# AVianEco/Softspoken

Measured on AMD Instinct MI355X. Metric: audio-seconds processed/sec (whole node), 16 kHz mono, higher is better.
Workload: dtype f16x2

## Files before the change

### softspoken_amd/csrc/conv4.hip

```cpp
#include "conv4_forms.h"
#include <cstdio>
#include <cstdlib>
#include <type_traits>
#include <utility>

namespace ss {

static constexpr int kMfmaPrio = 2;
__device__ __forceinline__ uint32_t relu_pk(uint32_t v) {
    return __builtin_bit_cast(uint32_t, __builtin_elementwise_max(__builtin_bit_cast(s16x2, v), s16x2{0, 0}));
}
__device__ __forceinline__ uint32_t max_pk(uint32_t a, uint32_t b) {
    return __builtin_bit_cast(uint32_t, __builtin_elementwise_max(__builtin_bit_cast(s16x2, a), __builtin_bit_cast(s16x2, b)));
}

template <int NT, int NW, bool BRES, bool RES, bool RADD, bool POOL, int RP, bool FIRST, bool FLAT, bool PF2, bool SPLIT = false, bool RANK1 = false,
          int NH = 1, bool GRES = false>
__global__ __launch_bounds__(64 * NW * NH) __attribute__((amdgpu_waves_per_eu((NT <= 2 && !(SPLIT && RES && !BRES && NW == 4 && NH == 1)) ? 4 : 2)))
void conv3x3_v4_kernel(ConvArgs a, int total_tiles, int lds_b_bytes) {
    constexpr int KC = 32;
    constexpr bool DUO = NH > 1;
    static_assert(!DUO || (NT == 1 && NW * NH == 16 && (RP == 0 || (GRES && RP == 1 && POOL)) && !FIRST && !FLAT && !PF2),
                  "DUO: the plain A / B launches; GRES also conv2_1.B's projection in B");
    static_assert(!GRES || (DUO && BRES && SPLIT && !RES), "GRES: f16x2 B launches with resident banks");
// ... 26 lines not shown
    const int hh = lane >> 5, m = lane & 31;
    const int py = (m >> 1) & 1, px = (m & 1) | ((m >> 2) << 1);
    char* sA = smem + half * kA;
    const int sb_bytes = RING ? 2 * lds_b_bytes : lds_b_bytes;
    char* sB = smem + NH * kA;
    const int proj_steps = RP ? (a.C0x + a.C1x) / 16 : 0;
    constexpr bool proj_lds = RP > 0 && (BRES || NT == 3 || SPLIT);
    const char* sProj = smem + NH * kA + sb_bytes;
    const int proj_tiles = SPLIT ? a.Cout / 32 : NT;
    const int proj_bank = proj_steps * proj_tiles * 1024;
    const float* sBias = (const float*)(sProj + (proj_lds ? (SPLIT ? 2 : 1) * proj_bank : 0));
    constexpr int FW = 20, FROWS = PR + 3;
    float* sFb = (float*)sBias + 32;
    float* sF = sFb + 32;
    float* sFlat = (float*)sBias + 32;

    const int H = a.H, W = a.W, Cout = a.Cout;
    const int ngroups = Cout / (32 * NT);
    const int nch_r = (a.C0 + a.C1) / KC;
    const int nch = SPLIT ? 2 * nch_r : nch_r;
    const int all_taps = nch_r * TAPS;

    const int xcd = blockIdx.x & 7, local = (int)(blockIdx.x >> 3) * NH + half, gper = (int)(gridDim.x >> 3) * NH;
    const int per = (total_tiles + 7) >> 3;
#ifdef SS_DEVBUILD
    const bool order_seq = !(a.dbg & 512);
#else
    constexpr bool order_seq = !kOrderSideBySide;
#endif
    auto tile_of = [&](int loc, int it) -> int {
        if constexpr (GRES) {
            const RingItem r = gres_item(xcd, loc / NH, (int)(gridDim.x >> 3), it, loc % NH, total_tiles / ngroups, ngroups, NH);
            return r.pos >= 0 ? r.pos * ngroups + r.g : -1;
        }
        if constexpr (RING) {
            const RingItem r = ring_item(xcd, loc / NH, (int)(gridDim.x >> 3), it, loc % NH, total_tiles / ngroups, ngroups, order_seq);
            return r.pos >= 0 ? r.pos * ngroups + r.g : -1;
        }
        const int idx = loc + it * gper;
        const int t = xcd * per + idx;
        return (idx < per && t < total_tiles) ? t : -1;
    };
    auto tile_at = [&](int it) -> int { return tile_of(local, it); };
    struct Tile { int n, y0, x0, g; };
    auto decode = [&](int t) -> Tile {
        Tile d;
        d.g = t % ngroups; t /= ngroups;
        d.x0 = (t % a.tiles_x) * 16; t /= a.tiles_x;
        d.y0 = (t % a.tiles_y) * TH;
        d.n = t / a.tiles_y;
        return d;
    };

    uint32_t pix_full[AIT], pix_half[AIT], lds_off[AIT], flags = 0;
    const uint32_t part16 = (tid & 3) * 16;
    {
        const int Wh = W >> 1;
#pragma unroll
        for (int it = 0; it < AIT; ++it) {
            const int p = tid + NTHR * it;
            const int pix = p >> 2;
            const int pyy = pix / kPatch, pxx = pix - pyy * kPatch;
            lds_off[it] = pyy * kRowPitch + pxx * kPixPitch + part16;
            pix_full[it] = pyy * W + pxx;
            pix_half[it] = ((pyy + 1) >> 1) * Wh + ((pxx + 1) >> 1);
            const uint32_t f = (pyy == 0 ? 1u : 0u) | (pyy == PR - 1 ? 2u : 0u) | (pxx == 0 ? 4u : 0u) | (pxx == kPatch - 1 ? 8u : 0u) |
                               (p >= NPA ? 16u : 0u);
            flags |= f << (8 * it);
        }
    }
    u32x4 ra0[AIT], ra1[AIT];
    u32x4 rb[BIT];
    float rf = 0.f;
    static_assert(!FIRST || (PR + 2) * FW <= NTHR, "one feature value per thread");

    auto issue_patch = [&](const Tile& d, int ci, u32x4 (&ra)[AIT]) {
        if constexpr (FIRST) {
            if constexpr (SPLIT) { if (ci & 1) return; }
            const int fy = tid / FW, fx = tid - fy * FW;
            const int Y = d.y0 - 2 + fy, X = d.x0 - 2 + fx;
            rf = (tid < (PR + 2) * FW && (unsigned)Y < (unsigned)H && (unsigned)X < (unsigned)W)
                     ? a.rank1_src[((size_t)d.n * H + Y) * W + X] : 0.f;
            return;
        }
        const int ch = (SPLIT ? ci >> 1 : ci) * KC;
        const int64_t plane = (SPLIT && !(ci & 1)) ? a.lo_delta : 0;
        const char* base; uint32_t cs2, toff; bool up;
        if (ch < a.C0) {
            base = (const char*)a.src0 - kHdr + plane; cs2 = 2u * a.C0; up = false;
            toff = kHdr + ((((uint32_t)d.n * H + d.y0 - 1) * W + d.x0 - 1) * a.C0 + ch) * 2u;
        } else {
            base = (const char*)a.src1 - kHdr + plane; cs2 = 2u * a.C1; up = true;
            toff = kHdr + ((((uint32_t)d.n * (H >> 1) + (d.y0 >> 1) - 1) * (W >> 1) + (d.x0 >> 1) - 1) * a.C1 + (ch - a.C0)) * 2u;
        }
        uint32_t tm = (d.y0 == 0 ? 1u : 0u) | (d.y0 + TH == H ? 2u : 0u) | (d.x0 == 0 ? 4u : 0u) | (d.x0 + 16 == W ? 8u : 0u) | 16u;
        const uint32_t tp = toff + part16;
#pragma unroll
        for (int it = 0; it < AIT; ++it) {
            const uint32_t pix = up ? pix_half[it] : pix_full[it];
            uint32_t off = __umul24(pix, cs2) + tp;
            if (flags & (tm << (8 * it))) off = 0;
            ra[it] = *(const u32x4*)(base + off);
        }
    };
    auto issue_weights = [&](const Tile& d, int ci) {
        if constexpr (!BRES && !RING) {
            if constexpr (SPLIT) { if (ci & 1) return; }
            const char* wsrc = SPLIT ? (const char*)a.wpk + ((size_t)d.g * nch_r + (ci >> 1)) * 2 * (TAPS * kTapBytes)
                                     : (const char*)a.wpk + ((size_t)d.g * all_taps + ci * TAPS) * kTapBytes;
#pragma unroll
            for (int it = 0; it < BIT; ++it) {
                const int p = tid + NTHR * it;
                u32x4 v = {0u, 0u, 0u, 0u};
                if (p < NPB) v = *(const u32x4*)(wsrc + p * 16);
                rb[it] = v;
            }
        }
    };
    auto commit = [&](u32x4 (&ra)[AIT], bool patch, bool bank) {
        if constexpr (FIRST) return;
        if (patch) {
#pragma unroll
            for (int it = 0; it < AIT; ++it) {
                if ((it + 1) * NTHR <= NPA || !(flags & (16u << (8 * it)))) *(u32x4*)(sA + lds_off[it]) = ra[it];
            }
        }
        if constexpr (!BRES && !RING) {
            if (bank) {
#pragma unroll
                for (int it = 0; it < BIT; ++it) {
                    const int p = tid + NTHR * it;
                    if (p < NPB) *(u32x4*)(sB + p * 16) = rb[it];
                }
            }
        }
    };
    constexpr int NPH = NPB / 2;
    const int ring_g0 = RING ? ring_group0((int)(blockIdx.x >> 3), ngroups, order_seq) : 0;
    const int ring_gstep = RING ? ring_group_step((int)(gridDim.x >> 3), ngroups, order_seq) : 0;
    int ring_g = ring_g0, ring_c = 0;
    auto ring_duty = [&](int s, int n_chunks) {
        if constexpr (RING) {
            if (half > 1) return;
            const int k = (s >> 1) + 1;
            if (k >= n_chunks) return;
            if (!(s & 1)) {
                if (++ring_c == nch_r) { ring_c = 0; ring_g += ring_gstep; if (ring_g >= ngroups) ring_g -= ngroups; }
                const char* wsrc = (const char*)a.wpk + ((size_t)(ring_g * nch_r + ring_c) * 2 + half) * (TAPS * kTapBytes);
#pragma unroll
                for (int it = 0; it < BIT; ++it) {
                    const int p = tid + NTHR * it;
                    u32x4 v = {0u, 0u, 0u, 0u};
// ... 267 lines not shown
                for (int nt = 0; nt < NT; ++nt) { rlo[nt] = *(const u32x4*)(rp + nt * 64); rhi[nt] = *(const u32x4*)(rp + nt * 64 + 32); }
            }
        }
        u32x4 fw[FLAT ? 2 : 1];
        u32x4 fw2[(FLAT && SPLIT) ? 2 : 1];
        auto load_flat_w = [&]() {
#pragma unroll
            for (int sx = 0; sx < 2; ++sx) {
                fw[sx] = *(const u32x4*)((const char*)a.flat_w4 + (((cur.y0 >> 1) + wave) * 2 + sx) * 1024 + lane * 16);
                if constexpr (SPLIT) fw2[sx] = *(const u32x4*)((const char*)a.flat_w4 + 64 * 2 * 1024 + (((cur.y0 >> 1) + wave) * 2 + sx) * 1024 + lane * 16);
            }
        };
        if constexpr (FLAT && !(SPLIT && RP > 0)) load_flat_w();
        u32x4 xf[RP ? RP : 1];
        if constexpr (RP > 0 && !SPLIT) {
            const uint32_t t_full = kHdr + ((((uint32_t)cur.n * H + cur.y0 + 2 * wave) * W + cur.x0) * a.C0x) * 2u;
            const uint32_t t_half = kHdr + ((((uint32_t)cur.n * (H >> 1) + (cur.y0 >> 1) + wave) * (W >> 1) + (cur.x0 >> 1)) * a.C1x) * 2u;
#pragma unroll
            for (int k = 0; k < RP; ++k) {
                const int sidx = ci * RP + k, ch = sidx * 16;
                const char* base; uint32_t off;
                if (sidx >= proj_steps) { base = (const char*)a.xp0 - kHdr; off = 0; }
                else if (ch < a.C0x) { base = (const char*)a.xp0 - kHdr; off = t_full + xf_off + ch * 2u; }
                else { base = (const char*)a.xp1 - kHdr; off = t_half + xh_off + (ch - a.C0x) * 2u; }
                xf[k] = *(const u32x4*)(base + off);
            }
        }
        u32x4 wpg[(RP && !proj_lds) ? RP : 1][NT];
        if constexpr (RP > 0 && !proj_lds && !SPLIT) {
            {
                const int tiles = Cout / 32;
#pragma unroll
                for (int k = 0; k < RP; ++k) {
                    const int sidx = ci * RP + k < proj_steps ? ci * RP + k : 0;
#pragma unroll
                    for (int nt = 0; nt < NT; ++nt)
                        wpg[k][nt] = *(const u32x4*)((const char*)a.proj_w + ((size_t)(sidx * tiles + cur.g * NT + nt) * 64 + lane) * 16);
                }
            }
        }
        if (ci == 0) {
#pragma unroll
            for (int nt = 0; nt < NT; ++nt)
#pragma unroll
                for (int g = 0; g < 4; ++g) {
                    const f32x4 b4 = *(const f32x4*)(sBias + co0 + nt * 32 + 8 * g + 4 * hh);
                    acc[nt][4 * g] = b4[0]; acc[nt][4 * g + 1] = b4[1]; acc[nt][4 * g + 2] = b4[2]; acc[nt][4 * g + 3] = b4[3];
                    if constexpr (RES) {
                        const f32x4 r4 = *(const f32x4*)(sBias + Cout + co0 + nt * 32 + 8 * g + 4 * hh);
                        racc[nt][4 * g] = r4[0]; racc[nt][4 * g + 1] = r4[1]; racc[nt][4 * g + 2] = r4[2]; racc[nt][4 * g + 3] = r4[3];
                    }
                }
        }
        auto proj_products = [&](auto k0c, auto k1c) {
            constexpr int K0 = decltype(k0c)::value, K1 = decltype(k1c)::value;
#pragma unroll
            for (int k = K0; k < K1; ++k) {
                const int sidx = (ci >> 1) * RP + k < proj_steps ? (ci >> 1) * RP + k : 0;
#pragma unroll
                for (int nt = 0; nt < NT; ++nt) {
                    const int wt = (sidx * proj_tiles + (int)(co0 >> 5) + nt) * 1024 + lane * 16;
                    const u32x4 wh = *(const u32x4*)(sProj + wt), wl = *(const u32x4*)(sProj + proj_bank + wt);
                    acc[nt] = mfma16<true>(wh, pxl[k - K0], acc[nt]);
                    acc[nt] = mfma16<true>(wl, pxh[k - K0], acc[nt]);
                    acc[nt] = mfma16<true>(wh, pxh[k - K0], acc[nt]);
                }
            }
        };
        using KZ_ = std::integral_constant<int, 0>; using KH_ = std::integral_constant<int, RPH>; using KR_ = std::integral_constant<int, RP>;
        if constexpr (SPLIT && RP > 0 && PART == 1) {
            proj_products(KZ_{}, KH_{});
            __builtin_amdgcn_sched_barrier(0);
            if constexpr (RP > RPH) issue_proj(cur, ci >> 1, KH_{}, KR_{});
        }
        if constexpr (FLAT && SPLIT && RP > 0) load_flat_w();
        {
            const char* bbase = sB + boff0 + (BRES ? ((DUO && !GRES ? cur.g * nch : 0) + (SPLIT ? (ci >> 1) * 2 : ci)) * TAPS * kTapBytes
                                                   : RING ? ((stage_no >> 1) & 1) * lds_b_bytes : 0);
            constexpr int PD = (NT == 1) ? 4 : 2;
            u32x4 af[PD], bfr[PD][NT];
            u32x4 rfr[RES ? 2 : 1][RES ? NT : 1];
            if (a.dbg & 32) __builtin_amdgcn_s_setprio(kMfmaPrio);
            constexpr bool kMerged = SPLIT && NSTEP == 36 && NT == 1;
            if constexpr (kMerged) {
                constexpr int PM = 3;
                u32x4 pf[PM], wh_[PM], wl_[PM], rh_[RES ? 2 : 1], rl_[RES ? 2 : 1];
                const char* bb0 = bbase; const char* bb1 = bbase + TAPS * kTapBytes;
                auto load3 = [&](int st, int slot) {
                    const int tap = st >> 1, sub = st & 1, dy = tap / 3, dx = tap % 3;
                    pf[slot] = *(const u32x4*)(sA + aoff0 + dy * kRowPitch + dx * kPixPitch + sub * 32);
                    wh_[slot] = *(const u32x4*)(bb0 + tap * kTapBytes + sub * 1024);
                    wl_[slot] = *(const u32x4*)(bb1 + tap * kTapBytes + sub * 1024);
                };
#pragma unroll
                for (int st = 0; st < PM - 1; ++st) load3(st, st);
#pragma unroll
                for (int st = 0; st < 18; ++st) {
                    if (st + PM - 1 < 18) load3(st + PM - 1, (st + PM - 1) % PM);
                    if constexpr (RES) {
                        if (st == 6) {
#pragma unroll
                            for (int sub = 0; sub < 2; ++sub) {
                                rh_[sub] = *(const u32x4*)(bb0 + 9 * kTapBytes + sub * 1024);
                                rl_[sub] = *(const u32x4*)(bb1 + 9 * kTapBytes + sub * 1024);
                            }
                        }
                    }
                    const u32x4 pixv = pf[st % PM];
                    acc[0] = mfma16<true>(wh_[st % PM], pixv, acc[0]);
                    acc[0] = mfma16<true>(wl_[st % PM], pixv, acc[0]);
                    if constexpr (RES) {
                        if (st == 8 || st == 9) {
                            racc[0] = mfma16<true>(rh_[st & 1], pixv, racc[0]);
                            racc[0] = mfma16<true>(rl_[st & 1], pixv, racc[0]);
                        }
                    }
                }
            } else
#pragma unroll
            for (int bank = 0; bank < NSTEP / 18; ++bank) {
                const char* bb = bbase + bank * TAPS * kTapBytes;
                auto load_frags = [&](int st, u32x4& fa, u32x4 (&fbb)[NT]) {
                    const int tap = st >> 1, sub = st & 1, dy = tap / 3, dx = tap % 3;
                    fa = *(const u32x4*)(sA + aoff0 + dy * kRowPitch + dx * kPixPitch + sub * 32);
#pragma unroll
                    for (int nt = 0; nt < NT; ++nt) fbb[nt] = *(const u32x4*)(bb + tap * kTapBytes + (sub * NT + nt) * 1024);
                };
                if (bank) __builtin_amdgcn_sched_barrier(0);
#pragma unroll
                for (int st = 0; st < PD - 1; ++st) load_frags(st, af[st], bfr[st]);
#pragma unroll
                for (int st = 0; st < 18; ++st) {
                    if (st + PD - 1 < 18) load_frags(st + PD - 1, af[(st + PD - 1) % PD], bfr[(st + PD - 1) % PD]);
                    if constexpr (RES) {
                        if (st == 6) {
#pragma unroll
                            for (int sub = 0; sub < 2; ++sub)
#pragma unroll
                                for (int nt = 0; nt < NT; ++nt) rfr[sub][nt] = *(const u32x4*)(bb + 9 * kTapBytes + (sub * NT + nt) * 1024);
                        }
                    }
                    const u32x4 pixv = af[st % PD];
#pragma unroll
                    for (int nt = 0; nt < NT; ++nt) {
                        acc[nt] = mfma16<SPLIT>(bfr[st % PD][nt], pixv, acc[nt]);
                        if constexpr (RES) {
                            if (st == 8 || st == 9) racc[nt] = mfma16<SPLIT>(rfr[st & 1][nt], pixv, racc[nt]);
                        }
                    }
                }
            }
        }

        if constexpr (SPLIT && RP > RPH && PART == 1) proj_products(KH_{}, KR_{});
        if constexpr (RP > 0 && !SPLIT) {
#pragma unroll
            for (int k = 0; k < RP; ++k) {
                const int sidx = ci * RP + k < proj_steps ? ci * RP + k : 0;
#pragma unroll
                for (int nt = 0; nt < NT; ++nt) {
                    u32x4 wp;
                    if constexpr (proj_lds) wp = *(const u32x4*)(sProj + (sidx * NT + nt) * 1024 + lane * 16); else wp = wpg[k][nt];
                    acc[nt] = __builtin_amdgcn_mfma_f32_32x32x16_bf16(__builtin_bit_cast(bf16x8, wp), __builtin_bit_cast(bf16x8, xf[k]), acc[nt], 0, 0, 0);
                }
            }
        }
        if (a.dbg & 32) __builtin_amdgcn_s_setprio(0);
        if constexpr (FIRST && !SPLIT) {
            const float f = sF[(2 * wave + py + 2) * FW + px + 2];
            const float fhi = (float)(__bf16)f, flo = f - fhi;
            u32x4 bop = {0u, 0u, 0u, 0u};
            if (hh == 0) { bop[0] = pack_bf16(fhi, flo); bop[1] = pack_bf16(fhi, 0.f); }
            acc[0] = __builtin_amdgcn_mfma_f32_32x32x16_bf16(__builtin_bit_cast(bf16x8, wr1), __builtin_bit_cast(bf16x8, bop), acc[0], 0, 0, 0);
        }
        auto epilogue = [&]() {
            __builtin_amdgcn_sched_barrier(0);
            if constexpr (SPLIT) {
#ifdef SS_DEVBUILD
                uint32_t te0 = 0;
                if (a.stamps) te0 = (uint32_t)__builtin_amdgcn_s_memtime();
#endif
                uint32_t ovf = 0;
                auto split_store = [&](const float (&v)[16], char* dst) {
                    Packed kh, kl;
    #pragma unroll
                    for (int g = 0; g < 4; ++g)
    #pragma unroll
                        for (int h = 0; h < 2; ++h) {
                            const float x0 = v[4 * g + 2 * h], x1 = v[4 * g + 2 * h + 1];
                            kh.p[g][h] = pack_f16(x0, x1);
                            ovf = pk_max_u16(ovf, kh.p[g][h]);
                            kl.p[g][h] = split_lo(kh.p[g][h], x0, x1);
                        }
                    return std::pair<Packed, Packed>(kh, kl);
                };
                if constexpr (RADD) {
    #pragma unroll
                    for (int nt = 0; nt < NT; ++nt) {
                        const f32x4 f0 = __builtin_bit_cast(f32x4, rlo[nt]), f1 = __builtin_bit_cast(f32x4, rhi[nt]);
                        const f32x4 f2 = __builtin_bit_cast(f32x4, rlo2[nt]), f3 = __builtin_bit_cast(f32x4, rhi2[nt]);
    #pragma unroll
                        for (int e = 0; e < 4; ++e) {
                            acc[nt][e] += f0[e];
                            acc[nt][4 + e] += f1[e];
                            acc[nt][8 + e] += f2[e];
                            acc[nt][12 + e] += f3[e];
                        }
// ... 330 lines not shown
```

### softspoken_amd/csrc/conv4_ups.hip

```cpp
#include "kernels.h"
#include "mfma_util.h"
#include <cstdlib>
#include <type_traits>

namespace ss {

namespace {

constexpr int kPix = 80;
constexpr int kRowR = 1472;
constexpr int kOdd = 720;
constexpr int kRowU = 896;
constexpr int kLowPlane = 6 * kRowU;
constexpr int kPatchBytes = 10 * kRowR;
constexpr int kBankR = 9 * 2048, kBankU = 16 * 2048;
constexpr int NW = 4, NH = 4, NTHR = 64 * NW;

}

__global__ __launch_bounds__(NTHR * NH) __attribute__((amdgpu_waves_per_eu(4)))
void conv3x3_ups_kernel(ConvArgs a, int total_tiles, int lds_b_bytes) {
    extern __shared__ __attribute__((aligned(16))) char smem[];
    const int half = __builtin_amdgcn_readfirstlane((int)threadIdx.x / NTHR);
    const int tid = (int)threadIdx.x % NTHR, lane = tid & 63;
// ... 103 lines not shown
        max_stages = n0 * nch;
        if (max_stages == 0) return;
    }
    Stage cs{0, decode(my_stages == 0 ? 0 : tile_of(local, 0))}, n1 = cs, n2 = cs;

    for (int p = (int)threadIdx.x; p < lds_b_bytes / 16; p += NTHR * NH) *(u32x4*)(sB + p * 16) = *(const u32x4*)((const char*)a.wpk + (size_t)p * 16);
    for (int i = (int)threadIdx.x; i < Cout; i += NTHR * NH) ((float*)sBias)[i] = a.bias[i];
    issue_patch(cs.d, 0);
    commit(0);
    bool ok1 = next_stage(cs, n1), ok2 = false;
    if (ok1) issue_patch(n1.d, n1.ci);
    __syncthreads();

    f32x16 acc;
    const int base_r = 2 * Y * kRowR + X * kPix + hh * 16;
    const int base_u = Y * kRowU + X * kPix + hh * 16;
    const int boff0 = lane * 16;
    const uint32_t st_off = (uint32_t)(((2 * Y + ca) * W + 2 * X + cb) * Cout + hh * 8) * 2u;
    int tap_r[9];
#pragma unroll
    for (int t = 0; t < 9; ++t) {
        const int dy = t / 3, dx = t % 3;
        tap_r[t] = (ca + dy) * kRowR + ((cb + dx) & 1) * kOdd + ((cb + dx) >> 1) * kPix;
    }
    int tap_u[4];
#pragma unroll
    for (int t = 0; t < 4; ++t) tap_u[t] = (ca + (t >> 1)) * kRowU + (cb + (t & 1)) * kPix;

    int jit_n = 0;
    auto jitter = [&](int site) {
#ifdef SS_DEVBUILD
        SS_JITTER_SLEEP(a.dbg, half * NW + wave, site, jit_n)
#else
        (void)site;
#endif
    };
    auto stage = [&]() -> bool {
        ++jit_n; jitter(0);
        const Tile cur = cs.d;
        const int ci = cs.ci;
        const bool last = ci == nch - 1;
        if (ci == 0) {
#pragma unroll
            for (int g = 0; g < 4; ++g) {
                const f32x4 b4 = *(const f32x4*)(sBias + 8 * g + 4 * hh);
                acc[4 * g] = b4[0]; acc[4 * g + 1] = b4[1]; acc[4 * g + 2] = b4[2]; acc[4 * g + 3] = b4[3];
            }
        }
        if (a.dbg & 32) __builtin_amdgcn_s_setprio(2);
        auto skip_stage = [&](auto part_c) {
            constexpr int PART = decltype(part_c)::value;
            const char* bb0 = sB + boff0 + (ci >> 1) * 2 * kBankR;
            const char* bb1 = bb0 + kBankR;
            constexpr int PM = 3;
            u32x4 pf[PM], wh_[PM], wl_[PM];
            auto load3 = [&](int st, int slot) {
                const int tap = st >> 1, sub = st & 1;
                pf[slot] = *(const u32x4*)(sA + base_r + tap_r[tap] + sub * 32);
                wh_[slot] = *(const u32x4*)(bb0 + tap * 2048 + sub * 1024);
                if constexpr (PART == 1) wl_[slot] = *(const u32x4*)(bb1 + tap * 2048 + sub * 1024);
            };
#pragma unroll
            for (int st = 0; st < PM - 1; ++st) load3(st, st);
#pragma unroll
            for (int st = 0; st < 18; ++st) {
                if (st + PM - 1 < 18) load3(st + PM - 1, (st + PM - 1) % PM);
                const u32x4 pixv = pf[st % PM];
                acc = mfma16<true>(wh_[st % PM], pixv, acc);
                if constexpr (PART == 1) acc = mfma16<true>(wl_[st % PM], pixv, acc);
            }
        };
        using P0 = std::integral_constant<int, 0>; using P1 = std::integral_constant<int, 1>;
        if (ci < 2 * nreg) {
            if (ci & 1) skip_stage(P1{}); else skip_stage(P0{});
        } else {
            const char* bb0 = sB + boff0 + nreg * 2 * kBankR + (ci - 2 * nreg) * 2 * kBankU + wave * 4 * 2048;
            const char* bb1 = bb0 + kBankU;
            constexpr int PM = 2;
            u32x4 ph[PM], pl[PM], wh_[PM], wl_[PM];
            auto load4 = [&](int st, int slot) {
                const int tap = st >> 1, sub = st & 1;
                ph[slot] = *(const u32x4*)(sA + base_u + tap_u[tap] + sub * 32);
                pl[slot] = *(const u32x4*)(sA + kLowPlane + base_u + tap_u[tap] + sub * 32);
                wh_[slot] = *(const u32x4*)(bb0 + tap * 2048 + sub * 1024);
                wl_[slot] = *(const u32x4*)(bb1 + tap * 2048 + sub * 1024);
            };
            load4(0, 0);
#pragma unroll
            for (int st = 0; st < 8; ++st) {
                if (st + 1 < 8) load4(st + 1, (st + 1) % PM);
                acc = mfma16<true>(wh_[st % PM], pl[st % PM], acc);
                acc = mfma16<true>(wl_[st % PM], ph[st % PM], acc);
                acc = mfma16<true>(wh_[st % PM], ph[st % PM], acc);
            }
        }
        if (a.dbg & 32) __builtin_amdgcn_s_setprio(0);
        jitter(1);
        lds_barrier();
        jitter(2);
        if (ok1) {
            commit(n1.ci);
            ok2 = next_stage(n1, n2);
            if (ok2) issue_patch(n2.d, n2.ci);
        }
        if (last) {
            __builtin_amdgcn_sched_barrier(0);
            uint32_t ovf = 0;
            Packed kh, kl;
#pragma unroll
            for (int g = 0; g < 4; ++g)
#pragma unroll
                for (int h = 0; h < 2; ++h) {
                    const float x0 = relu_i(acc[4 * g + 2 * h]), x1 = relu_i(acc[4 * g + 2 * h + 1]);
                    kh.p[g][h] = pack_f16(x0, x1);
                    ovf = pk_max_u16(ovf, kh.p[g][h]);
                    kl.p[g][h] = split_lo(kh.p[g][h], x0, x1);
                }
            char* op = (char*)a.out + ((((uint32_t)cur.n * H + cur.y0) * W + cur.x0) * Cout) * 2u + st_off;
            u32x4 lo, hi;
            to_runs(kh, lo, hi);
            *(u32x4*)(op) = lo;
            *(u32x4*)(op + 32) = hi;
            to_runs(kl, lo, hi);
            *(u32x4*)(op + a.lo_delta) = lo;
            *(u32x4*)(op + a.lo_delta + 32) = hi;
            if (((ovf & 0x7fff7fffu) + 0x04000400u) & 0x80008000u) atomicOr(a.range_flag, 1);
        }
        jitter(3);
        lds_barrier();
        jitter(4);
        cs = n1; n1 = n2;
        const bool more = ok1;
        ok1 = ok1 && ok2;
        return more;
    };
    for (int i = 0; i < half; ++i) lds_barrier();
    for (int s = 0; s < max_stages; ++s) {
        if (s < my_stages) stage();
        else { lds_barrier(); lds_barrier(); }
    }
    for (int i = half; i < NH - 1; ++i) lds_barrier();
}

namespace {
constexpr int kEntR = 10 * 2048;
constexpr int kEntRH = kEntR + 256;
// ... 111 lines not shown
            ra[1] = *(const u32x4*)(base + (off ? a.lo_delta + off : 0));
        }
    };
    auto commit = [&](int sec) {
        if (sec == 0) {
#pragma unroll
            for (int it = 0; it < AIT; ++it)
                if (!(flags & (16u << (8 * it)))) *(u32x4*)(sA + lds_off[it]) = ra[it];
        } else if (!(flags_low & 16u)) {
            *(u32x4*)(sA + lds_low) = ra[0];
            *(u32x4*)(sA + kLowPlane + lds_low) = ra[1];
        }
    };

    Tile cur = decode_pos(my_items ? ring_item(xcd, wg, nwg, 0, half, total_pos, ngroups, order_seq).pos : 0, g0), nxt = cur;
    int cur_i = 0, nxt_i = 0;
    bool nxt_ok = false;
    auto compute_next = [&]() {
        nxt_i = cur_i + 1;
        nxt_ok = nxt_i < my_items;
        if (nxt_ok) { const RingItem r = ring_item(xcd, wg, nwg, nxt_i, half, total_pos, ngroups, order_seq); nxt = decode_pos(r.pos, r.g); }
    };
    struct Cur { Sp sp; Tile d; bool ok; };
    auto advance = [&](Cur& c) {
        if (sp_next(c.sp)) { c.d = nxt; c.ok = nxt_ok; }
    };
    Cur ip{Sp{0, 0, 0}, cur, true};

    {
        Sp p{0, 0, 0};
        for (int e = 0; e < 3; ++e) {
            const char* src = (const char*)a.wpk + (size_t)g0 * group_bytes + entry_off(p);
            const int np = entry_size(p) / 16;
            for (int q = (int)threadIdx.x; q < np; q += NTHR * NH) *(u32x4*)(sR + e * kSlot + q * 16) = *(const u32x4*)(src + (size_t)q * 16);
            do sp_next(p); while (!starts_entry(p));
        }
    }
    Sp rq{0, 0, 0};
    int rq_g = g0, rq_t = 0, rq_e = 0, rq_slot = 0;
    auto rq_advance = [&]() {
        if (starts_entry(rq)) { ++rq_e; rq_slot = rq_slot == 2 ? 0 : rq_slot + 1; }
        ++rq_t;
        if (sp_next(rq)) { rq_g += gstep; if (rq_g >= ngroups) rq_g -= ngroups; }
    };
    if (half & 1) for (int i = 0; i < (half == 1 ? 2 : 3); ++i) rq_advance();
    auto ring_issue = [&]() {
        if (!(half & 1)) return;
        if (!SS_ABL(19) && rq_t < max_stages && rq_e >= 3 && starts_entry(rq)) {
            const int total = entry_size(rq) / 16;
            const int h0 = ((total / 2 + 63) / 64) * 64;
            const int base = half == 1 ? 0 : h0, cnt = half == 1 ? h0 : total - h0;
            const char* src = (const char*)a.wpk + (size_t)rq_g * group_bytes + entry_off(rq) + base * 16;
            char* dst = sR + rq_slot * kSlot + base * 16 + wave * 1024;
#pragma unroll
            for (int it = 0; it < kGL; ++it) {
                const int idx = tid + NTHR * it;
                if (idx < cnt)
                    __builtin_amdgcn_global_load_lds((const __attribute__((address_space(1))) void*)(src + (size_t)idx * 16),
                                                     (__attribute__((address_space(3))) void*)(uintptr_t)(dst + it * NTHR * 16), 16, 0, 0);
            }
        }
        rq_advance();
    };

    issue_patch(ip.d, ip.sp);
    commit(0);
    if (my_stages == 0) ip.ok = false;
    else do advance(ip); while (ip.ok && !needs_patch(ip.sp));
    if (ip.ok) issue_patch(ip.d, ip.sp);
    __syncthreads();

    f32x16 acc, racc;
    auto mm = [&](const u32x4& w, const u32x4& x, const f32x16& c) -> f32x16 { return SS_ABL(16) ? c : mfma16<true>(w, x, c); };
    const int base_r = 2 * Y * kRowR + X * kPix + hh * 16;
    const int base_u = Y * kRowU + X * kPix + hh * 16;
    const int boff0 = lane * 16;
    const uint32_t st_off = (uint32_t)(((2 * Y + ca) * W + 2 * X + cb) * Cout + hh * 8) * 2u;
    const uint32_t r_lane = (uint32_t)(32 * hh + 4 * X + 2 * ca + cb) * 32u;
    int tap_r[9];
#pragma unroll
    for (int t = 0; t < 9; ++t) {
        const int dy = t / 3, dx = t % 3;
        tap_r[t] = (ca + dy) * kRowR + ((cb + dx) & 1) * kOdd + ((cb + dx) >> 1) * kPix;
    }
    int tap_u[4];
#pragma unroll
    for (int t = 0; t < 4; ++t) tap_u[t] = (ca + (t >> 1)) * kRowU + (cb + (t & 1)) * kPix;
    constexpr int kCentreU = kRowU + kPix;

    int jit_n = 0;
#ifdef SS_DEVBUILD
    uint32_t st_prev = 0, st_sub = 0, st_sum[9] = {0u, 0u, 0u, 0u, 0u, 0u, 0u, 0u, 0u};
#endif
    auto substamp = [&](int seg) {
#ifdef SS_DEVBUILD
        if (a.stamps) { const uint32_t t = (uint32_t)__builtin_amdgcn_s_memtime(); if (seg >= 5) st_sum[seg] += t - st_sub; st_sub = t; }
#else
        (void)seg;
#endif
    };
    auto jitter = [&](int site) {
#ifdef SS_DEVBUILD
        if (a.stamps) {
            const uint32_t t = (uint32_t)__builtin_amdgcn_s_memtime();
            const int seg = site == 0 ? 4 : site - 1;
            if (site != 0 || jit_n > 1) st_sum[seg] += t - st_prev;
            st_prev = t;
        }
        SS_JITTER_SLEEP(a.dbg, half * NW + wave, site, jit_n)
#else
        (void)site;
// ... 4 lines not shown
    bool have_done = false;
    auto store_h = [&]() {
        __builtin_amdgcn_sched_barrier(0);
        uint32_t ovf = 0;
        Packed kh, kl;
#pragma unroll
        for (int g = 0; g < 4; ++g)
#pragma unroll
            for (int h = 0; h < 2; ++h) {
                const float x0 = relu_i(acc_done[4 * g + 2 * h]), x1 = relu_i(acc_done[4 * g + 2 * h + 1]);
                kh.p[g][h] = pack_f16(x0, x1);
                ovf = pk_max_u16(ovf, kh.p[g][h]);
                kl.p[g][h] = split_lo(kh.p[g][h], x0, x1);
            }
        char* op = (char*)a.out + done_off * 2u + st_off;
        u32x4 lo, hi;
        to_runs(kh, lo, hi);
        *(u32x4*)(op) = lo;
        *(u32x4*)(op + 32) = hi;
        to_runs(kl, lo, hi);
        *(u32x4*)(op + a.lo_delta) = lo;
        *(u32x4*)(op + a.lo_delta + 32) = hi;
        if (((ovf & 0x7fff7fffu) + 0x04000400u) & 0x80008000u) atomicOr(a.range_flag, 1);
        __builtin_amdgcn_sched_barrier(0);
    };
    int e_slot = 0;
    int stage_no = 0;
    auto stage = [&](auto kind_c, int c) {
        constexpr int KIND = decltype(kind_c)::value;
        ++jit_n; jitter(0);
        const bool last = nups ? (KIND == 4 && c == nups - 1) : (KIND == 2 && c == nreg - 1);
        const char* ent = sR + e_slot * kSlot;
        if (KIND == 0 && c == 0) {
            const float* sBias = (const float*)(ent + kEntR);
#pragma unroll
            for (int g = 0; g < 4; ++g) {
                const f32x4 b4 = *(const f32x4*)(sBias + 8 * g + 4 * hh);
                const f32x4 r4 = *(const f32x4*)(sBias + 32 + 8 * g + 4 * hh);
                acc[4 * g] = b4[0]; acc[4 * g + 1] = b4[1]; acc[4 * g + 2] = b4[2]; acc[4 * g + 3] = b4[3];
                racc[4 * g] = r4[0]; racc[4 * g + 1] = r4[1]; racc[4 * g + 2] = r4[2]; racc[4 * g + 3] = r4[3];
            }
        }
        if (a.dbg & 32) __builtin_amdgcn_s_setprio(2);
        if constexpr (KIND <= 2) {
            const char* bb = ent + boff0;
            constexpr int PM = 3;
            u32x4 pf[PM], wf[PM];
            auto load2 = [&](int st, int slot) {
                if (SS_ABL(17)) return;
                const int tap = st >> 1, sub = st & 1;
                pf[slot] = *(const u32x4*)(sA + base_r + tap_r[tap] + sub * 32);
                wf[slot] = *(const u32x4*)(bb + tap * 2048 + sub * 1024);
            };
            u32x4 wr0, wr1;
#pragma unroll
            for (int st = 0; st < PM - 1; ++st) load2(st, st);
#pragma unroll
            for (int st = 0; st < 18; ++st) {
                if (st + PM - 1 < 18) load2(st + PM - 1, (st + PM - 1) % PM);
                if (st == 6) wr0 = *(const u32x4*)(bb + 9 * 2048);
                if (st == 7) wr1 = *(const u32x4*)(bb + 9 * 2048 + 1024);
                acc = mm(wf[st % PM], pf[st % PM], acc);
                if (st == 8) racc = mm(wr0, pf[st % PM], racc);
                if (st == 9) racc = mm(wr1, pf[st % PM], racc);
            }
        } else if constexpr (KIND == 3) {
            const char* bb = ent + boff0 + wave * 4 * 2048;
            constexpr int PM = 2;
            u32x4 ph[PM], pl[PM], wf[PM];
            auto load3 = [&](int st, int slot) {
                if (SS_ABL(17)) return;
                const int tap = st >> 1, sub = st & 1;
                ph[slot] = *(const u32x4*)(sA + base_u + tap_u[tap] + sub * 32);
                pl[slot] = *(const u32x4*)(sA + kLowPlane + base_u + tap_u[tap] + sub * 32);
                wf[slot] = *(const u32x4*)(bb + tap * 2048 + sub * 1024);
            };
            load3(0, 0);
#pragma unroll
            for (int st = 0; st < 8; ++st) {
                if (st + 1 < 8) load3(st + 1, (st + 1) % PM);
                acc = mm(wf[st % PM], pl[st % PM], acc);
                acc = mm(wf[st % PM], ph[st % PM], acc);
            }
#pragma unroll
            for (int sub = 0; sub < 2; ++sub) {
                const u32x4 w = *(const u32x4*)(ent + boff0 + 16 * 2048 + sub * 1024);
                const u32x4 xh = *(const u32x4*)(sA + base_u + kCentreU + sub * 32), xl = *(const u32x4*)(sA + kLowPlane + base_u + kCentreU + sub * 32);
                racc = mm(w, xl, racc);
                racc = mm(w, xh, racc);
            }
        } else {
            const char* bb = ent + boff0 + wave * 4 * 2048;
            constexpr int PM = 3;
            u32x4 ph[PM], wf[PM];
            auto load2 = [&](int st, int slot) {
                if (SS_ABL(17)) return;
                const int tap = st >> 1, sub = st & 1;
                ph[slot] = *(const u32x4*)(sA + base_u + tap_u[tap] + sub * 32);
                wf[slot] = *(const u32x4*)(bb + tap * 2048 + sub * 1024);
            };
#pragma unroll
            for (int st = 0; st < PM - 1; ++st) load2(st, st);
#pragma unroll
            for (int st = 0; st < 8; ++st) {
                if (st + PM - 1 < 8) load2(st + PM - 1, (st + PM - 1) % PM);
                acc = mm(wf[st % PM], ph[st % PM], acc);
            }
#pragma unroll
            for (int sub = 0; sub < 2; ++sub) {
                const u32x4 w = *(const u32x4*)(ent + boff0 + 16 * 2048 + sub * 1024);
                const u32x4 xh = *(const u32x4*)(sA + base_u + kCentreU + sub * 32);
                racc = mm(w, xh, racc);
            }
        }
        if (a.dbg & 32) __builtin_amdgcn_s_setprio(0);
        jitter(1);
        vm_lds_barrier();
        jitter(2);
        const bool more = stage_no + 1 < my_stages;
        constexpr bool next_has_patch = KIND == 0 || KIND == 2 || KIND == 4;
        const int next_sec = KIND == 0 ? 0 : KIND == 2 ? ((c == nreg - 1 && nups) ? 1 : 0) : (c == nups - 1 ? 0 : 1);
        const bool np = next_has_patch && more;
        substamp(0);
        if (np) commit(next_sec);
        substamp(5);
        if (last && !SS_ABL(20)) {
            char* rq_p = (char*)a.res_out +
                         ((((((uint32_t)cur.n * (H >> 1) + (cur.y0 >> 1) + Y) * (W >> 4) + (cur.x0 >> 4)) * (uint32_t)ngroups) + cur.g) * 2048u + r_lane);
            *(f32x4*)(rq_p) = f32x4{racc[0], racc[1], racc[2], racc[3]};
            *(f32x4*)(rq_p + 16) = f32x4{racc[4], racc[5], racc[6], racc[7]};
            *(f32x4*)(rq_p + a.lo_delta) = f32x4{racc[8], racc[9], racc[10], racc[11]};
            *(f32x4*)(rq_p + a.lo_delta + 16) = f32x4{racc[12], racc[13], racc[14], racc[15]};
        }
        if (last) { acc_done = acc; done_off = (((uint32_t)cur.n * H + cur.y0) * W + cur.x0) * Cout + cur.g * 32; have_done = true; }
        if (KIND == 1 && c == 0 && have_done && !SS_ABL(20)) { store_h(); have_done = false; }
        if (KIND == 1 && c == 0) compute_next();
        if (last && more) { cur = nxt; cur_i = nxt_i; }
        substamp(6);
        if (np) {
            do advance(ip); while (ip.ok && !needs_patch(ip.sp));
            if (ip.ok) issue_patch(ip.d, ip.sp);
        }
        substamp(7);
        ring_issue();
        substamp(8);
        jitter(3);
        lds_barrier();
        jitter(4);
        if (KIND != 0) e_slot = e_slot == 2 ? 0 : e_slot + 1;
        ++stage_no;
    };
    using K0 = std::integral_constant<int, 0>; using K1 = std::integral_constant<int, 1>; using K2 = std::integral_constant<int, 2>;
    using K3 = std::integral_constant<int, 3>; using K4 = std::integral_constant<int, 4>;
    const int my_pg = my_items, max_pg = max_stages / nst;
    for (int i = 0; i < half; ++i) lds_barrier();
    for (int pg = 0; pg < max_pg; ++pg) {
        if (pg < my_pg) {
            for (int c = 0; c < nreg; ++c) { stage(K0{}, c); stage(K1{}, c); stage(K2{}, c); }
            for (int c = 0; c < nups; ++c) { stage(K3{}, c); stage(K4{}, c); }
        } else {
            for (int st = 0; st < nst; ++st) { vm_lds_barrier(); ring_issue(); lds_barrier(); }
        }
    }
    for (int i = half; i < NH - 1; ++i) lds_barrier();
    if (have_done && !SS_ABL(20)) store_h();
// ... 107 lines not shown
```

### softspoken_amd/csrc/mfma_util.h

```cpp
#pragma once
#include <hip/hip_runtime.h>
#include <stdint.h>

namespace ss {

typedef float f32x16 __attribute__((ext_vector_type(16)));
typedef float f32x4 __attribute__((ext_vector_type(4)));
typedef float f32x2 __attribute__((ext_vector_type(2)));
typedef __bf16 bf16x8 __attribute__((ext_vector_type(8)));
typedef __bf16 bf16x2 __attribute__((ext_vector_type(2)));
typedef _Float16 f16x8 __attribute__((ext_vector_type(8)));
typedef _Float16 f16x2 __attribute__((ext_vector_type(2)));
typedef short s16x2 __attribute__((ext_vector_type(2)));
typedef uint32_t u32x4 __attribute__((ext_vector_type(4)));
typedef uint32_t u32x2 __attribute__((ext_vector_type(2)));

static constexpr int kHdr = 256;

__device__ __forceinline__ void wave_lds_sync() { asm volatile("s_waitcnt lgkmcnt(0)" ::: "memory"); }
__device__ __forceinline__ void lds_barrier() { asm volatile("s_waitcnt lgkmcnt(0)\n\ts_barrier" ::: "memory"); }
__device__ __forceinline__ void vm_lds_barrier() { asm volatile("s_waitcnt vmcnt(0) lgkmcnt(0)\n\ts_barrier" ::: "memory"); }

__device__ __forceinline__ uint32_t pack_bf16(float lo, float hi) {
    return __builtin_bit_cast(uint32_t, __builtin_convertvector(f32x2{lo, hi}, bf16x2));
}
__device__ __forceinline__ uint32_t pack_f16(float lo, float hi) {
    return __builtin_bit_cast(uint32_t, __builtin_convertvector(f32x2{lo, hi}, f16x2));
}
__device__ __forceinline__ f32x2 unpack_f16(uint32_t v) { return __builtin_convertvector(__builtin_bit_cast(f16x2, v), f32x2); }
__device__ __forceinline__ uint32_t pk_max_u16(uint32_t a, uint32_t b) {
    uint32_t r;
    asm("v_pk_max_u16 %0, %1, %2" : "=v"(r) : "v"(a), "v"(b));
    return r;
}
__device__ __forceinline__ uint32_t split_lo(uint32_t hi, float x0, float x1) {
    uint32_t l;
    asm("v_fma_mixlo_f16 %0, %1, -1.0, %2 op_sel_hi:[1,0,0]" : "=v"(l) : "v"(hi), "v"(x0));
    asm("v_fma_mixhi_f16 %0, %1, -1.0, %2 op_sel:[1,0,0] op_sel_hi:[1,0,0]" : "+v"(l) : "v"(hi), "v"(x1));
    return l;
}
__device__ __forceinline__ float relu_i(float x) {
    const int b = __builtin_bit_cast(int, x);
    return __builtin_bit_cast(float, b > 0 ? b : 0);
}
template <bool F16>
__device__ __forceinline__ f32x16 mfma16(const u32x4& a, const u32x4& b, const f32x16& c) {
    if constexpr (F16) return __builtin_amdgcn_mfma_f32_32x32x16_f16(__builtin_bit_cast(f16x8, a), __builtin_bit_cast(f16x8, b), c, 0, 0, 0);
    else return __builtin_amdgcn_mfma_f32_32x32x16_bf16(__builtin_bit_cast(bf16x8, a), __builtin_bit_cast(bf16x8, b), c, 0, 0, 0);
}
__device__ __forceinline__ void half_swap(uint32_t& x, uint32_t& y) {
    const u32x2 r = __builtin_amdgcn_permlane32_swap(x, y, false, false);
    x = r[0]; y = r[1];
}

struct Packed { uint32_t p[4][2]; };

__device__ __forceinline__ void to_runs(Packed& k, u32x4& lo, u32x4& hi) {
    half_swap(k.p[0][0], k.p[1][0]); half_swap(k.p[0][1], k.p[1][1]);
    half_swap(k.p[2][0], k.p[3][0]); half_swap(k.p[2][1], k.p[3][1]);
    lo = u32x4{k.p[0][0], k.p[0][1], k.p[1][0], k.p[1][1]};
    hi = u32x4{k.p[2][0], k.p[2][1], k.p[3][0], k.p[3][1]};
}
__device__ __forceinline__ void from_runs(const u32x4& lo, const u32x4& hi, Packed& k) {
    k.p[0][0] = lo[0]; k.p[0][1] = lo[1]; k.p[1][0] = lo[2]; k.p[1][1] = lo[3];
    k.p[2][0] = hi[0]; k.p[2][1] = hi[1]; k.p[3][0] = hi[2]; k.p[3][1] = hi[3];
    half_swap(k.p[0][0], k.p[1][0]); half_swap(k.p[0][1], k.p[1][1]);
    half_swap(k.p[2][0], k.p[3][0]); half_swap(k.p[2][1], k.p[3][1]);
}

}

#define SS_JITTER_SLEEP(dbg, wave, site, n)                                                                                               \
    if ((dbg) & 1024) {                                                                                                                   \
        const int pat_ = ((dbg) >> 11) & 3, w_ = (wave);                                                                                  \
        const bool z_ = pat_ == 0 ? ((w_ + (site) + (n)) & 3) == 0 : pat_ == 1 ? w_ == 0 : pat_ == 2 ? w_ != 0 : (w_ & 1) != 0;           \
        if (z_) __builtin_amdgcn_s_sleep(32);                                                                                             \
    }
```

Before: 31010.

## Cut VGPR pressure in conv MFMA loops with sched fences and shallower prefetch

Adds a sched_barrier-based frag_fence around MFMA steps and reduces the LDS fragment prefetch depth in the split/merged paths. Projection-weight loads are double-buffered, and one of them can be issued early. Residual weight fragments are loaded one at a time instead of held in pairs. Drops the unused pix_half array for no-upsample variants and streamlines the global_load_lds address math. The goal is lower register pressure and more predictable interleaving of LDS loads and MFMAs, at the risk of exposing LDS latency and constraining the compiler's scheduler.

```diff
diff --git a/softspoken_amd/csrc/conv4.hip b/softspoken_amd/csrc/conv4.hip
--- a/softspoken_amd/csrc/conv4.hip
+++ b/softspoken_amd/csrc/conv4.hip
@@ -102,7 +102,8 @@
         return d;
     };
 
-    uint32_t pix_full[AIT], pix_half[AIT], lds_off[AIT], flags = 0;
+    constexpr bool kNoUp = FIRST || FLAT || RANK1;
+    uint32_t pix_full[AIT], pix_half[kNoUp ? 1 : AIT], lds_off[AIT], flags = 0;
     const uint32_t part16 = (tid & 3) * 16;
     {
         const int Wh = W >> 1;
@@ -113,7 +114,7 @@
             const int pyy = pix / kPatch, pxx = pix - pyy * kPatch;
             lds_off[it] = pyy * kRowPitch + pxx * kPixPitch + part16;
             pix_full[it] = pyy * W + pxx;
-            pix_half[it] = ((pyy + 1) >> 1) * Wh + ((pxx + 1) >> 1);
+            if constexpr (!kNoUp) pix_half[it] = ((pyy + 1) >> 1) * Wh + ((pxx + 1) >> 1);
             const uint32_t f = (pyy == 0 ? 1u : 0u) | (pyy == PR - 1 ? 2u : 0u) | (pxx == 0 ? 4u : 0u) | (pxx == kPatch - 1 ? 8u : 0u) |
                                (p >= NPA ? 16u : 0u);
             flags |= f << (8 * it);
@@ -136,7 +137,7 @@
         const int ch = (SPLIT ? ci >> 1 : ci) * KC;
         const int64_t plane = (SPLIT && !(ci & 1)) ? a.lo_delta : 0;
         const char* base; uint32_t cs2, toff; bool up;
-        if (ch < a.C0) {
+        if (kNoUp || ch < a.C0) {
             base = (const char*)a.src0 - kHdr + plane; cs2 = 2u * a.C0; up = false;
             toff = kHdr + ((((uint32_t)d.n * H + d.y0 - 1) * W + d.x0 - 1) * a.C0 + ch) * 2u;
         } else {
@@ -147,7 +148,7 @@
         const uint32_t tp = toff + part16;
 #pragma unroll
         for (int it = 0; it < AIT; ++it) {
-            const uint32_t pix = up ? pix_half[it] : pix_full[it];
+            const uint32_t pix = (!kNoUp && up) ? pix_half[kNoUp ? 0 : it] : pix_full[it];
             uint32_t off = __umul24(pix, cs2) + tp;
             if (flags & (tm << (8 * it))) off = 0;
             ra[it] = *(const u32x4*)(base + off);
@@ -521,24 +522,34 @@
                     }
                 }
         }
-        auto proj_products = [&](auto k0c, auto k1c) {
+        u32x4 pwh[2], pwl[2];
+        auto proj_load = [&](auto k0c, int j) {
+            constexpr int K0 = decltype(k0c)::value;
+            const int k = K0 + j / NT, nt = j % NT;
+            const int sidx = (ci >> 1) * RP + k < proj_steps ? (ci >> 1) * RP + k : 0;
+            const int wt = (sidx * proj_tiles + (int)(co0 >> 5) + nt) * 1024 + lane * 16;
+            pwh[j & 1] = *(const u32x4*)(sProj + wt); pwl[j & 1] = *(const u32x4*)(sProj + proj_bank + wt);
+        };
+        auto proj_products = [&](auto k0c, auto k1c, auto early_c) {
             constexpr int K0 = decltype(k0c)::value, K1 = decltype(k1c)::value;
-#pragma unroll
-            for (int k = K0; k < K1; ++k) {
-                const int sidx = (ci >> 1) * RP + k < proj_steps ? (ci >> 1) * RP + k : 0;
-#pragma unroll
-                for (int nt = 0; nt < NT; ++nt) {
-                    const int wt = (sidx * proj_tiles + (int)(co0 >> 5) + nt) * 1024 + lane * 16;
-                    const u32x4 wh = *(const u32x4*)(sProj + wt), wl = *(const u32x4*)(sProj + proj_bank + wt);
-                    acc[nt] = mfma16<true>(wh, pxl[k - K0], acc[nt]);
-                    acc[nt] = mfma16<true>(wl, pxh[k - K0], acc[nt]);
-                    acc[nt] = mfma16<true>(wh, pxh[k - K0], acc[nt]);
-                }
+            constexpr int NJ = (K1 - K0) * NT;
+            if constexpr (NJ > 0 && !decltype(early_c)::value) proj_load(k0c, 0);
+            frag_fence();
+#pragma unroll
+            for (int j = 0; j < NJ; ++j) {
+                const int k = K0 + j / NT, nt = j % NT;
+                if (j + 1 < NJ) proj_load(k0c, j + 1);
+                frag_fence();
+                acc[nt] = mfma16<true>(pwh[j & 1], pxl[k - K0], acc[nt]);
+                acc[nt] = mfma16<true>(pwl[j & 1], pxh[k - K0], acc[nt]);
+                acc[nt] = mfma16<true>(pwh[j & 1], pxh[k - K0], acc[nt]);
+                frag_fence();
             }
         };
+        constexpr bool kProjEarly = SPLIT && RP > RPH && PART == 1 && NSTEP == 36 && NT == 1 && !(NW == 4 && NH == 1 && !BRES);
         using KZ_ = std::integral_constant<int, 0>; using KH_ = std::integral_constant<int, RPH>; using KR_ = std::integral_constant<int, RP>;
         if constexpr (SPLIT && RP > 0 && PART == 1) {
-            proj_products(KZ_{}, KH_{});
+            proj_products(KZ_{}, KH_{}, std::false_type{});
             __builtin_amdgcn_sched_barrier(0);
             if constexpr (RP > RPH) issue_proj(cur, ci >> 1, KH_{}, KR_{});
         }
@@ -546,14 +557,16 @@
         {
             const char* bbase = sB + boff0 + (BRES ? ((DUO && !GRES ? cur.g * nch : 0) + (SPLIT ? (ci >> 1) * 2 : ci)) * TAPS * kTapBytes
                                                    : RING ? ((stage_no >> 1) & 1) * lds_b_bytes : 0);
-            constexpr int PD = (NT == 1) ? 4 : 2;
+            constexpr bool kFence = SPLIT && !(NW == 4 && NH == 1 && !BRES);
+            auto fence = [&]() { if constexpr (kFence) frag_fence(); };
+            constexpr int PD = (NT == 1) ? (kFence ? 3 : 4) : 2;
             u32x4 af[PD], bfr[PD][NT];
             u32x4 rfr[RES ? 2 : 1][RES ? NT : 1];
             if (a.dbg & 32) __builtin_amdgcn_s_setprio(kMfmaPrio);
             constexpr bool kMerged = SPLIT && NSTEP == 36 && NT == 1;
             if constexpr (kMerged) {
-                constexpr int PM = 3;
-                u32x4 pf[PM], wh_[PM], wl_[PM], rh_[RES ? 2 : 1], rl_[RES ? 2 : 1];
+                constexpr int PM = kFence ? 2 : 3;
+                u32x4 pf[PM], wh_[PM], wl_[PM], rh_, rl_;
                 const char* bb0 = bbase; const char* bb1 = bbase + TAPS * kTapBytes;
                 auto load3 = [&](int st, int slot) {
                     const int tap = st >> 1, sub = st & 1, dy = tap / 3, dx = tap % 3;
@@ -563,27 +576,29 @@
                 };
 #pragma unroll
                 for (int st = 0; st < PM - 1; ++st) load3(st, st);
+                fence();
 #pragma unroll
                 for (int st = 0; st < 18; ++st) {
                     if (st + PM - 1 < 18) load3(st + PM - 1, (st + PM - 1) % PM);
+                    if constexpr (kProjEarly) { if (st == 17) proj_load(KH_{}, 0); }
                     if constexpr (RES) {
-                        if (st == 6) {
-#pragma unroll
-                            for (int sub = 0; sub < 2; ++sub) {
-                                rh_[sub] = *(const u32x4*)(bb0 + 9 * kTapBytes + sub * 1024);
-                                rl_[sub] = *(const u32x4*)(bb1 + 9 * kTapBytes + sub * 1024);
-                            }
-                        }
-                    }
+                        if (st == 6 || st == 9) {
+                            rh_ = *(const u32x4*)(bb0 + 9 * kTapBytes + (st == 9) * 1024);
+                            rl_ = *(const u32x4*)(bb1 + 9 * kTapBytes + (st == 9) * 1024);
+                        }
+                    }
+                    fence();
                     const u32x4 pixv = pf[st % PM];
                     acc[0] = mfma16<true>(wh_[st % PM], pixv, acc[0]);
                     acc[0] = mfma16<true>(wl_[st % PM], pixv, acc[0]);
                     if constexpr (RES) {
                         if (st == 8 || st == 9) {
-                            racc[0] = mfma16<true>(rh_[st & 1], pixv, racc[0]);
-                            racc[0] = mfma16<true>(rl_[st & 1], pixv, racc[0]);
-                        }
-                    }
+                            fence();
+                            racc[0] = mfma16<true>(rh_, pixv, racc[0]);
+                            racc[0] = mfma16<true>(rl_, pixv, racc[0]);
+                        }
+                    }
+                    fence();
                 }
             } else
 #pragma unroll
@@ -598,6 +613,7 @@
                 if (bank) __builtin_amdgcn_sched_barrier(0);
 #pragma unroll
                 for (int st = 0; st < PD - 1; ++st) load_frags(st, af[st], bfr[st]);
+                fence();
 #pragma unroll
                 for (int st = 0; st < 18; ++st) {
                     if (st + PD - 1 < 18) load_frags(st + PD - 1, af[(st + PD - 1) % PD], bfr[(st + PD - 1) % PD]);
@@ -609,6 +625,7 @@
                                 for (int nt = 0; nt < NT; ++nt) rfr[sub][nt] = *(const u32x4*)(bb + 9 * kTapBytes + (sub * NT + nt) * 1024);
                         }
                     }
+                    fence();
                     const u32x4 pixv = af[st % PD];
 #pragma unroll
                     for (int nt = 0; nt < NT; ++nt) {
@@ -617,11 +634,12 @@
                             if (st == 8 || st == 9) racc[nt] = mfma16<SPLIT>(rfr[st & 1][nt], pixv, racc[nt]);
                         }
                     }
-                }
-            }
-        }
-
-        if constexpr (SPLIT && RP > RPH && PART == 1) proj_products(KH_{}, KR_{});
+                    fence();
+                }
+            }
+        }
+
+        if constexpr (SPLIT && RP > RPH && PART == 1) proj_products(KH_{}, KR_{}, std::bool_constant<kProjEarly>{});
         if constexpr (RP > 0 && !SPLIT) {
 #pragma unroll
             for (int k = 0; k < RP; ++k) {
diff --git a/softspoken_amd/csrc/conv4_ups.hip b/softspoken_amd/csrc/conv4_ups.hip
--- a/softspoken_amd/csrc/conv4_ups.hip
+++ b/softspoken_amd/csrc/conv4_ups.hip
@@ -179,7 +179,7 @@
             constexpr int PART = decltype(part_c)::value;
             const char* bb0 = sB + boff0 + (ci >> 1) * 2 * kBankR;
             const char* bb1 = bb0 + kBankR;
-            constexpr int PM = 3;
+            constexpr int PM = PART == 1 ? 2 : 3;
             u32x4 pf[PM], wh_[PM], wl_[PM];
             auto load3 = [&](int st, int slot) {
                 const int tap = st >> 1, sub = st & 1;
@@ -189,12 +189,15 @@
             };
 #pragma unroll
             for (int st = 0; st < PM - 1; ++st) load3(st, st);
+            frag_fence();
 #pragma unroll
             for (int st = 0; st < 18; ++st) {
                 if (st + PM - 1 < 18) load3(st + PM - 1, (st + PM - 1) % PM);
+                frag_fence();
                 const u32x4 pixv = pf[st % PM];
                 acc = mfma16<true>(wh_[st % PM], pixv, acc);
                 if constexpr (PART == 1) acc = mfma16<true>(wl_[st % PM], pixv, acc);
+                frag_fence();
             }
         };
         using P0 = std::integral_constant<int, 0>; using P1 = std::integral_constant<int, 1>;
@@ -213,12 +216,15 @@
                 wl_[slot] = *(const u32x4*)(bb1 + tap * 2048 + sub * 1024);
             };
             load4(0, 0);
+            frag_fence();
 #pragma unroll
             for (int st = 0; st < 8; ++st) {
                 if (st + 1 < 8) load4(st + 1, (st + 1) % PM);
+                frag_fence();
                 acc = mfma16<true>(wh_[st % PM], pl[st % PM], acc);
                 acc = mfma16<true>(wl_[st % PM], ph[st % PM], acc);
                 acc = mfma16<true>(wh_[st % PM], ph[st % PM], acc);
+                frag_fence();
             }
         }
         if (a.dbg & 32) __builtin_amdgcn_s_setprio(0);
@@ -436,11 +442,12 @@
             const int base = half == 1 ? 0 : h0, cnt = half == 1 ? h0 : total - h0;
             const char* src = (const char*)a.wpk + (size_t)rq_g * group_bytes + entry_off(rq) + base * 16;
             char* dst = sR + rq_slot * kSlot + base * 16 + wave * 1024;
+            uint32_t t16 = (uint32_t)tid * 16u;
+            asm volatile("" : "+v"(t16));
 #pragma unroll
             for (int it = 0; it < kGL; ++it) {
-                const int idx = tid + NTHR * it;
-                if (idx < cnt)
-                    __builtin_amdgcn_global_load_lds((const __attribute__((address_space(1))) void*)(src + (size_t)idx * 16),
+                if (tid < cnt - NTHR * it)
+                    __builtin_amdgcn_global_load_lds((const __attribute__((address_space(1))) void*)(src + (size_t)(t16 + (uint32_t)(it * NTHR * 16))),
                                                      (__attribute__((address_space(3))) void*)(uintptr_t)(dst + it * NTHR * 16), 16, 0, 0);
             }
         }
@@ -551,17 +558,15 @@
                 pf[slot] = *(const u32x4*)(sA + base_r + tap_r[tap] + sub * 32);
                 wf[slot] = *(const u32x4*)(bb + tap * 2048 + sub * 1024);
             };
-            u32x4 wr0, wr1;
+            u32x4 wr;
 #pragma unroll
             for (int st = 0; st < PM - 1; ++st) load2(st, st);
 #pragma unroll
             for (int st = 0; st < 18; ++st) {
                 if (st + PM - 1 < 18) load2(st + PM - 1, (st + PM - 1) % PM);
-                if (st == 6) wr0 = *(const u32x4*)(bb + 9 * 2048);
-                if (st == 7) wr1 = *(const u32x4*)(bb + 9 * 2048 + 1024);
+                if ((st == 7 || st == 9) && !SS_ABL(17)) wr = *(const u32x4*)(bb + 9 * 2048 + (st == 9) * 1024);
                 acc = mm(wf[st % PM], pf[st % PM], acc);
-                if (st == 8) racc = mm(wr0, pf[st % PM], racc);
-                if (st == 9) racc = mm(wr1, pf[st % PM], racc);
+                if (st == 8 || st == 9) racc = mm(wr, pf[st % PM], racc);
             }
         } else if constexpr (KIND == 3) {
             const char* bb = ent + boff0 + wave * 4 * 2048;
@@ -574,19 +579,24 @@
                 pl[slot] = *(const u32x4*)(sA + kLowPlane + base_u + tap_u[tap] + sub * 32);
                 wf[slot] = *(const u32x4*)(bb + tap * 2048 + sub * 1024);
             };
+            auto load_r = [&](int sub, int slot) {
+                if (SS_ABL(17)) return;
+                wf[slot] = *(const u32x4*)(ent + boff0 + 16 * 2048 + sub * 1024);
+                ph[slot] = *(const u32x4*)(sA + base_u + kCentreU + sub * 32);
+                pl[slot] = *(const u32x4*)(sA + kLowPlane + base_u + kCentreU + sub * 32);
+            };
             load3(0, 0);
 #pragma unroll
             for (int st = 0; st < 8; ++st) {
-                if (st + 1 < 8) load3(st + 1, (st + 1) % PM);
+                if (st + 1 < 8) load3(st + 1, (st + 1) % PM); else load_r(0, (st + 1) % PM);
                 acc = mm(wf[st % PM], pl[st % PM], acc);
                 acc = mm(wf[st % PM], ph[st % PM], acc);
             }
 #pragma unroll
             for (int sub = 0; sub < 2; ++sub) {
-                const u32x4 w = *(const u32x4*)(ent + boff0 + 16 * 2048 + sub * 1024);
-                const u32x4 xh = *(const u32x4*)(sA + base_u + kCentreU + sub * 32), xl = *(const u32x4*)(sA + kLowPlane + base_u + kCentreU + sub * 32);
-                racc = mm(w, xl, racc);
-                racc = mm(w, xh, racc);
+                if (sub == 0) load_r(1, 1);
+                racc = mm(wf[sub], pl[sub], racc);
+                racc = mm(wf[sub], ph[sub], racc);
             }
         } else {
             const char* bb = ent + boff0 + wave * 4 * 2048;
@@ -598,18 +608,19 @@
                 ph[slot] = *(const u32x4*)(sA + base_u + tap_u[tap] + sub * 32);
                 wf[slot] = *(const u32x4*)(bb + tap * 2048 + sub * 1024);
             };
-#pragma unroll
-            for (int st = 0; st < PM - 1; ++st) load2(st, st);
-#pragma unroll
-            for (int st = 0; st < 8; ++st) {
-                if (st + PM - 1 < 8) load2(st + PM - 1, (st + PM - 1) % PM);
-                acc = mm(wf[st % PM], ph[st % PM], acc);
-            }
-#pragma unroll
-            for (int sub = 0; sub < 2; ++sub) {
-                const u32x4 w = *(const u32x4*)(ent + boff0 + 16 * 2048 + sub * 1024);
-                const u32x4 xh = *(const u32x4*)(sA + base_u + kCentreU + sub * 32);
-                racc = mm(w, xh, racc);
+            auto load_any = [&](int st, int slot) {
+                if (st < 8) { load2(st, slot); return; }
+                if (SS_ABL(17)) return;
+                wf[slot] = *(const u32x4*)(ent + boff0 + 16 * 2048 + (st - 8) * 1024);
+                ph[slot] = *(const u32x4*)(sA + base_u + kCentreU + (st - 8) * 32);
+            };
+#pragma unroll
+            for (int st = 0; st < PM - 1; ++st) load_any(st, st);
+#pragma unroll
+            for (int st = 0; st < 10; ++st) {
+                if (st + PM - 1 < 10) load_any(st + PM - 1, (st + PM - 1) % PM);
+                if (st < 8) acc = mm(wf[st % PM], ph[st % PM], acc);
+                else racc = mm(wf[st % PM], ph[st % PM], racc);
             }
         }
         if (a.dbg & 32) __builtin_amdgcn_s_setprio(0);
diff --git a/softspoken_amd/csrc/mfma_util.h b/softspoken_amd/csrc/mfma_util.h
--- a/softspoken_amd/csrc/mfma_util.h
+++ b/softspoken_amd/csrc/mfma_util.h
@@ -48,6 +48,7 @@
     if constexpr (F16) return __builtin_amdgcn_mfma_f32_32x32x16_f16(__builtin_bit_cast(f16x8, a), __builtin_bit_cast(f16x8, b), c, 0, 0, 0);
     else return __builtin_amdgcn_mfma_f32_32x32x16_bf16(__builtin_bit_cast(bf16x8, a), __builtin_bit_cast(bf16x8, b), c, 0, 0, 0);
 }
+__device__ __forceinline__ void frag_fence() { __builtin_amdgcn_sched_barrier(0); }
 __device__ __forceinline__ void half_swap(uint32_t& x, uint32_t& y) {
     const u32x2 r = __builtin_amdgcn_permlane32_swap(x, y, false, false);
     x = r[0]; y = r[1];
```

Measured after the change: 31430, median of 6. 1.01x the previous value.
